# kuldeepbrd1/graspLDM

Hardware: AMD Instinct MI355X
Metric: grasps/sec whole-node (1024-pt cloud, 100 DDIM steps) (higher is better)
Workload: dtype f32 (GEMMs as split-f16 x3 partial products on the f16 matrix pipe, f32 accumulation; GroupNorm / LayerNorm / attention / scheduler in f32); 1 GPU; LDM mode, 256 synthetic 1024-pt clouds per GPU x 20 grasps, 100 DDIM steps: BASELINE.json configs[2] per GPU (configs[3] = this per-GPU workload on 8 GPUs); experiment=fpc, clouds_per_gpu=256, grasps_per_cloud=20, points=1024, ddim_steps=100, encoder=PVCNNEncoder (shipped fpc config), parallelism=cloud-sharded x1, weights=synthetic recipe seed 0, streams=3

## Files before the change

graspldm_amd/csrc/pointwise_mlp.hip:

```cpp
#include "mfma_core.h"

namespace {

struct PwArgs {
  const float *x, *w, *bias, *head_w, *head_b;
  float *y, *z;
  int cin, cout, n, relu, hout, tiles_per_cloud, total_tiles;
  const float *w0, *bias0;
  int cin0;
  int dyn_first;
  int ticket_off;
  int x0_in_planes;
  const float *add;
  long long add_bs, add_rs, add_cs;
  int ranged, rng_off;
  float gain0_r, gain0_b;
  int y_point_major;
  int cin_rows;
};

__global__ __launch_bounds__(512, 2) void pointwise_mlp_kernel(const PwArgs a) {
  constexpr int NC = 32;
  extern __shared__ float lds[];
  const int tid = threadIdx.x, lane = tid & 63;
  const int wave = __builtin_amdgcn_readfirstlane(tid >> 6);
  Ctx c{a.w, lds, tid, wave, lane, 0, 2};
  const int col = lane & 15, kq = lane >> 4;
  const int cblocks = a.cin >> 4, mtiles = a.cout >> 4, mt_per_wave = mtiles >> 3;
  float *zpart = lds + a.cin * NC;
  const WStream hw(a.head_w ? a.head_w : a.w, lane);
  for (int tile = blockIdx.x; tile < a.total_tiles; tile += gridDim.x) {
    const int b = tile / a.tiles_per_cloud, c0 = (tile - b * a.tiles_per_cloud) * NC;
    __syncthreads();
    if (a.w0) {
      float *x0 = zpart + 8 * 16 * NC;
      const float *xb0 = a.x + (size_t)b * a.cin0 * a.n + c0;
      for (int i = tid; i < a.cin0 * 8; i += 512) {
        const int row = i >> 3, q = i & 7;
        *reinterpret_cast<f32x4 *>(x0 + swz<NC>(row, 4 * q)) = *reinterpret_cast<const f32x4 *>(xb0 + (size_t)row * a.n + 4 * q);
      }
      __syncthreads();
      const int cb0 = a.cin0 >> 4, mt_per_wave0 = a.cin >> 7;
      for (int ps = 0; ps < mt_per_wave0; ps += 2) {
        const int mt0 = wave * mt_per_wave0 + ps;
        f32x4 acc[2][2];
#pragma unroll
        for (int mi = 0; mi < 2; ++mi) {
          const f32x4 bv = *reinterpret_cast<const f32x4 *>(a.bias0 + 16 * (mt0 + mi) + 4 * kq);
          acc[mi][0] = bv;
          acc[mi][1] = bv;
        }
        gemm_fast_pf<NC, 4, 1, 2, 2, 2>(c, a.w0, cb0, mt0, 0, x0, acc);
        lds_f *d3 = (lds_f *)lds;
#pragma unroll
        for (int mi = 0; mi < 2; ++mi)
#pragma unroll
          for (int r = 0; r < 4; ++r)
#pragma unroll
            for (int ni = 0; ni < 2; ++ni)
              d3[swz<NC>(16 * (mt0 + mi) + 4 * kq + r, 16 * ni + col)] = fmaxf(acc[mi][ni][r], 0.f);
      }
    } else {
      const float *xb = a.x + (size_t)b * a.cin * a.n + c0;
      for (int i = tid; i < a.cin * 8; i += 512) {
        const int row = i >> 3, q = i & 7;
        const f32x4 v = *reinterpret_cast<const f32x4 *>(xb + (size_t)row * a.n + 4 * q);
        *reinterpret_cast<f32x4 *>(lds + swz<NC>(row, 4 * q)) = v;
      }
    }
    __syncthreads();
    f32x4 zacc[2] = {f32x4{0.f, 0.f, 0.f, 0.f}, f32x4{0.f, 0.f, 0.f, 0.f}};
    for (int ps = 0; ps < mt_per_wave; ps += 2) {
      const int mt0 = wave * mt_per_wave + ps;
      f32x4 acc[2][2];
#pragma unroll
      for (int mi = 0; mi < 2; ++mi) {
        const f32x4 bv = *reinterpret_cast<const f32x4 *>(a.bias + 16 * (mt0 + mi) + 4 * kq);
        acc[mi][0] = bv;
        acc[mi][1] = bv;
      }
      if ((cblocks & 3) == 0) gemm_fast_pf<NC, 4, 1, 2, 2, 4>(c, a.w, cblocks, mt0, 0, lds, acc);
      else gemm_fast_pf<NC, 4, 1, 2, 2, 2>(c, a.w, cblocks, mt0, 0, lds, acc);
#pragma unroll
      for (int mi = 0; mi < 2; ++mi) {
        if (a.relu) {
#pragma unroll
          for (int ni = 0; ni < 2; ++ni)
#pragma unroll
            for (int r = 0; r < 4; ++r) acc[mi][ni][r] = fmaxf(acc[mi][ni][r], 0.f);
        }
        if (a.y) {
          float *yb = a.y + ((size_t)b * a.cout + 16 * (mt0 + mi) + 4 * kq) * a.n + c0 + col;
#pragma unroll
          for (int r = 0; r < 4; ++r)
#pragma unroll
            for (int ni = 0; ni < 2; ++ni) __builtin_nontemporal_store(acc[mi][ni][r], yb + (size_t)r * a.n + 16 * ni);
        }
        if (a.head_w) {
          const f32x4 ah = hw[(size_t)(mt0 + mi) * 64];
#pragma unroll
          for (int r = 0; r < 4; ++r)
#pragma unroll
            for (int ni = 0; ni < 2; ++ni)
              zacc[ni] = __builtin_amdgcn_mfma_f32_16x16x4f32(ah[r], acc[mi][ni][r], zacc[ni], 0, 0, 0);
        }
      }
    }
    if (a.head_w) {
#pragma unroll
      for (int ni = 0; ni < 2; ++ni)
#pragma unroll
        for (int r = 0; r < 4; ++r) zpart[(wave * 16 + 4 * kq + r) * NC + 16 * ni + col] = zacc[ni][r];
      __syncthreads();
      for (int i = tid; i < a.hout * NC; i += 512) {
        const int row = i / NC, cc = i - row * NC;
        float v = a.head_b ? a.head_b[row] : 0.f;
#pragma unroll
        for (int w8 = 0; w8 < 8; ++w8) v += zpart[(w8 * 16 + row) * NC + cc];
        a.z[((size_t)b * a.hout + row) * a.n + c0 + cc] = v;
      }
    }
  }
}

template <int NC>
__device__ __forceinline__ int pw_swz(int row, int col) { return row * NC + (col < 32 ? (col ^ ((row & 1) << 4)) : col); }
template <int NC>
__device__ __forceinline__ void store_planes4_pw(float *planes, int c0, int n, float v0, float v1, float v2, float v3) {
  unsigned h0, h1, l0, l1;
  split_f16x2(v0, v1, h0, l0);
  split_f16x2(v2, v3, h1, l1);
  const int a = ((((c0 >> 5) * kSplit) * 4 + ((c0 >> 3) & 3)) * NC + n) * 4 + ((c0 >> 2) & 1) * 2;
  lds_u2 *d = (lds_u2 *)(planes + a);
  d[0] = u32x2_t{h0, h1};
  d[8 * NC] = u32x2_t{l0, l1};
}

template <int KB0, int NT>
__device__ __forceinline__ void pw_front_split(const WStream &w0s, const float *bias0, const float *x0, float *planes,
                                               int wave, int lane, int mt_per_wave0, bool x0_in_planes, float bsc, float osc) {
  constexpr int NC = 16 * NT;
  const int col = lane & 15, kq = lane >> 4;
  u32x4 bp[KB0][NT][kSplit];
#pragma unroll
  for (int kb = 0; kb < KB0; ++kb)
#pragma unroll
    for (int ni = 0; ni < NT; ++ni) {
      float v[8];
#pragma unroll
      for (int j = 0; j < 8; ++j) v[j] = x0[pw_swz<NC>(32 * kb + 8 * kq + j, 16 * ni + col)] * bsc;
      split_planes8(v, bp[kb][ni]);
    }
  if (x0_in_planes) __syncthreads();
  u32x4 af[2][KB0][kSplit];
  const int mt_first = wave * mt_per_wave0, mt_last = mt_first + mt_per_wave0 - 2;
  auto load_a = [&](int mi, int kb, int mt0) {
#pragma unroll
    for (int pl = 0; pl < kSplit; ++pl) af[mi][kb][pl] = w0s.raw_at(((mt0 + mi) * KB0 + kb) * kFragBytes, pl * 1024);
  };
#pragma unroll
  for (int mi = 0; mi < 2; ++mi)
#pragma unroll
    for (int kb = 0; kb < KB0; ++kb) load_a(mi, kb, mt_first);
  for (int mt0 = mt_first; mt0 <= mt_last; mt0 += 2) {
    const int mtn = mt0 + 2 <= mt_last ? mt0 + 2 : mt_last;
    f32x4 acc[2][NT];
#pragma unroll
    for (int mi = 0; mi < 2; ++mi) {
      const f32x4 bv = *reinterpret_cast<const f32x4 *>(bias0 + 16 * (mt0 + mi) + 4 * kq) * bsc;
#pragma unroll
      for (int ni = 0; ni < NT; ++ni) acc[mi][ni] = bv;
    }
#pragma unroll
    for (int mi = 0; mi < 2; ++mi)
#pragma unroll
      for (int kb = 0; kb < KB0; ++kb) {
#pragma unroll
        for (int ni = 0; ni < NT; ++ni) acc[mi][ni] = mfma_split(af[mi][kb], bp[kb][ni], acc[mi][ni]);
        __builtin_amdgcn_sched_barrier(0);
        load_a(mi, kb, mtn);
        __builtin_amdgcn_sched_barrier(0);
      }
#pragma unroll
    for (int mi = 0; mi < 2; ++mi)
#pragma unroll
      for (int ni = 0; ni < NT; ++ni)
        store_planes4_pw<NC>(planes, 16 * (mt0 + mi) + 4 * kq, 16 * ni + col, fmaxf(acc[mi][ni][0], 0.f) * osc,
                             fmaxf(acc[mi][ni][1], 0.f) * osc, fmaxf(acc[mi][ni][2], 0.f) * osc, fmaxf(acc[mi][ni][3], 0.f) * osc);
  }
}

#ifdef GLDM_DEBUG_KNOBS
__device__ long long g_pw_stamp[64];
#define GLDM_PW_STAMP(i) \
  do { if (blockIdx.x == 5 && tile == 5 + 2 * (int)gridDim.x && (threadIdx.x & 63) == 0 && (wave == 0 || wave == 7)) \
         g_pw_stamp[(wave ? 32 : 0) + (i)] = (long long)__builtin_readcyclecounter(); } while (0)
#else
#define GLDM_PW_STAMP(i) do {} while (0)
#endif
template <bool ADD, int NT, int MU = 2>
__global__ __launch_bounds__(512, 2) void pointwise_mlp_sp_kernel(const PwArgs a) {
  constexpr int NC = 16 * NT;
  extern __shared__ float lds[];
  const int tid = threadIdx.x, lane = tid & 63;
  const int wave = __builtin_amdgcn_readfirstlane(tid >> 6);
  const int col = lane & 15, kq = lane >> 4;
  const int kb32 = a.cin >> 5, mtiles = a.cout >> 4;
  float *planes = lds;
  float *zpart = lds;
  float *zdyn = lds + a.cin * (NC / 2) * kSplit;
  float *x0 = a.x0_in_planes ? lds : zdyn;
  int *ticket = (int *)(lds + a.ticket_off);
  const WStream hw(a.head_w ? a.head_w : a.w, lane);
  const WStream wv(a.w, lane);
  const lds_u4 *pl3 = (const lds_u4 *)planes + kq * NC + col;
  for (int tile = blockIdx.x; tile < a.total_tiles; tile += gridDim.x) {
    const int b = tile / a.tiles_per_cloud, c0 = (tile - b * a.tiles_per_cloud) * NC;
    const int ntv = min(NT, (a.n - c0) >> 4);
    __syncthreads();
    GLDM_PW_STAMP(0);
    if (tid == 0) *ticket = a.dyn_first;
    float s_main = 1.0f;
    float *rng = lds + a.rng_off;
    auto range_publish = [&](float mx) {
      mx = half_max(row_pair_max(row16_max(mx)));
      if (lane == 0) rng[wave] = mx;
    };
    auto range_read = [&]() {
      const f32x4 r0 = *reinterpret_cast<const f32x4 *>(rng), r1 = *reinterpret_cast<const f32x4 *>(rng + 4);
      const float mx = fmaxf(fmaxf(fmaxf(r0[0], r0[1]), fmaxf(r0[2], r0[3])), fmaxf(fmaxf(r1[0], r1[1]), fmaxf(r1[2], r1[3])));
      return __uint_as_float(__builtin_amdgcn_readfirstlane(__float_as_uint(mx)));
    };
    if (a.w0) {
      const float *xb0 = a.x + (size_t)b * a.cin0 * a.n + c0;
      float mx = 0.f;
      for (int i = tid; i < a.cin0 * (NC / 4); i += 512) {
        const int row = i / (NC / 4), q = i - row * (NC / 4);
        f32x4 v = f32x4{0.f, 0.f, 0.f, 0.f};
        if (4 * q < 16 * ntv) v = *reinterpret_cast<const f32x4 *>(xb0 + (size_t)row * a.n + 4 * q);
        *reinterpret_cast<f32x4 *>(x0 + pw_swz<NC>(row, 4 * q)) = v;
        mx = fmaxf(fmaxf(mx, fmaxf(fabsf(v[0]), fabsf(v[1]))), fmaxf(fabsf(v[2]), fabsf(v[3])));
      }
      if (a.ranged) range_publish(mx);
      __syncthreads();
      GLDM_PW_STAMP(1);
      float bsc = 1.0f, osc = 1.0f;
      if (a.ranged) {
        const float m0 = range_read(), s0 = range_pow2(m0);
        s_main = range_pow2(a.gain0_r * m0 + a.gain0_b);
        bsc = pow2_inv(s0);
        osc = s0 * pow2_inv(s_main);
      }
      const int mt_per_wave0 = a.cin >> 7;
      const WStream w0s(a.w0, lane);
      switch (a.cin0 >> 5) {
        case 1: pw_front_split<1, NT>(w0s, a.bias0, x0, planes, wave, lane, mt_per_wave0, a.x0_in_planes != 0, bsc, osc); break;
        case 2: pw_front_split<2, NT>(w0s, a.bias0, x0, planes, wave, lane, mt_per_wave0, a.x0_in_planes != 0, bsc, osc); break;
        default: pw_front_split<3, NT>(w0s, a.bias0, x0, planes, wave, lane, mt_per_wave0, a.x0_in_planes != 0, bsc, osc); break;
      }
    } else {
      const float *xb = a.x + (size_t)b * a.cin_rows * a.n + c0;
      constexpr int kHold = 2;
      const int items = (a.cin >> 3) * NC;
      auto stage_store = [&](int i, float (&v)[8], float inv) {
        const int kg = i / NC, scol = i - kg * NC, row = 8 * kg;
#pragma unroll
        for (int j = 0; j < 8; ++j) v[j] *= inv;
        u32x4 pl[kSplit];
        split_planes8(v, pl);
        lds_u4 *d = (lds_u4 *)planes + (((row >> 5) * kSplit) * 4 + ((row >> 3) & 3)) * NC + scol;
        d[0] = pl[0];
        d[4 * NC] = pl[1];
      };
      auto stage_load = [&](int i, float (&v)[8]) {
        const int kg = i / NC, scol = i - kg * NC, row = 8 * kg;
        const bool in = scol < 16 * ntv && row < a.cin_rows;
#pragma unroll
        for (int j = 0; j < 8; ++j) v[j] = in ? xb[(size_t)(row + j) * a.n + scol] : 0.f;
      };
      if (NT == 2 && a.ranged && items <= kHold * 512) {
        float hv[kHold][8];
        float mx = 0.f;
#pragma unroll
        for (int q = 0; q < kHold; ++q) {
          const int i = tid + 512 * q;
          if (i < items) {
            stage_load(i, hv[q]);
#pragma unroll
            for (int j = 0; j < 8; ++j) mx = fmaxf(mx, fabsf(hv[q][j]));
          }
        }
        range_publish(mx);
        __syncthreads();
        s_main = range_pow2(range_read());
        const float inv = pow2_inv(s_main);
#pragma unroll
        for (int q = 0; q < kHold; ++q) {
          const int i = tid + 512 * q;
          if (i < items) stage_store(i, hv[q], inv);
        }
      } else {
        float inv = 1.0f;
        if (a.ranged) {
          float mx = 0.f;
          for (int i = tid; i < items; i += 512) {
            float v[8];
            stage_load(i, v);
#pragma unroll
            for (int j = 0; j < 8; ++j) mx = fmaxf(mx, fabsf(v[j]));
          }
          range_publish(mx);
          __syncthreads();
          s_main = range_pow2(range_read());
          inv = pow2_inv(s_main);
        }
        for (int i = tid; i < items; i += 512) {
          float v[8];
          stage_load(i, v);
          stage_store(i, v, inv);
        }
      }
    }
    GLDM_PW_STAMP(2);
    __syncthreads();
    GLDM_PW_STAMP(3);
    f32x4 zacc[NT];
#pragma unroll
    for (int ni = 0; ni < NT; ++ni) zacc[ni] = f32x4{0.f, 0.f, 0.f, 0.f};
    const int units = mtiles / MU;
    u32x4 af[4][MU][kSplit];
    auto load_a = [&](int buf, int mt0, int kb) {
#pragma unroll
      for (int mi = 0; mi < MU; ++mi)
#pragma unroll
        for (int pl = 0; pl < kSplit; ++pl) af[buf][mi][pl] = wv.raw_at(((mt0 + mi) * kb32 + kb) * kFragBytes, pl * 1024);
    };
    u32x4 bs[2][NT][kSplit];
    auto load_b = [&](int buf, int kb) {
#pragma unroll
      for (int ni = 0; ni < NT; ++ni)
#pragma unroll
        for (int pl = 0; pl < kSplit; ++pl) bs[buf][ni][pl] = pl3[(kb * kSplit + pl) * 4 * NC + 16 * ni];
    };
    auto draw = [&]() {
      int t = 0;
      if (lane == 0) t = __hip_atomic_fetch_add(ticket, 1, __ATOMIC_RELAXED, __HIP_MEMORY_SCOPE_WORKGROUP);
      return __builtin_amdgcn_readfirstlane(t);
    };
    const int dyn_first = a.dyn_first;
    int unit = wave;
#pragma unroll
    for (int u = 0; u < 4; ++u) load_a(u, MU * (unit < units ? unit : 0), u);
    load_b(0, 0);
    while (unit < units) {
      const int mt0 = MU * unit;
      const int nxt = unit + 8 < dyn_first ? unit + 8 : draw();
      const int mtn = MU * (nxt < units ? nxt : unit);
      f32x4 acc[MU][NT], bv[MU], ah[MU];
#pragma unroll
      for (int mi = 0; mi < MU; ++mi) {
        bv[mi] = *reinterpret_cast<const f32x4 *>(a.bias + 16 * (mt0 + mi) + 4 * kq);
        ah[mi] = hw[(size_t)(a.head_w ? mt0 + mi : 0) * 64];
#pragma unroll
        for (int ni = 0; ni < NT; ++ni) acc[mi][ni] = f32x4{0.f, 0.f, 0.f, 0.f};
      }
      for (int kb0 = 0; kb0 < kb32; kb0 += 4) {
        const bool tail = kb0 + 4 >= kb32;
#pragma unroll
        for (int u = 0; u < 4; ++u) {
          const int kb = kb0 + u;
          load_b((u + 1) & 1, kb + 1 < kb32 ? kb + 1 : 0);
          __builtin_amdgcn_sched_barrier(0);
#pragma unroll
          for (int mi = 0; mi < MU; ++mi)
#pragma unroll
            for (int ni = 0; ni < NT; ++ni) acc[mi][ni] = mfma_split(af[u][mi], bs[u & 1][ni], acc[mi][ni]);
          __builtin_amdgcn_sched_barrier(0);
          load_a(u, tail ? mtn : mt0, tail ? u : kb + 4);
        }
      }
#pragma unroll
      for (int mi = 0; mi < MU; ++mi) {
#pragma unroll
        for (int ni = 0; ni < NT; ++ni)
#pragma unroll
          for (int r = 0; r < 4; ++r) {
            float v = __builtin_fmaf(acc[mi][ni][r], s_main, bv[mi][r]);
            if constexpr (ADD)
              v += a.add[(long long)b * a.add_bs + (long long)(16 * (mt0 + mi) + 4 * kq + r) * a.add_rs +
                         (long long)(c0 + (ni < ntv ? 16 * ni + col : col)) * a.add_cs];
            acc[mi][ni][r] = a.relu ? fmaxf(v, 0.f) : v;
          }
        if (a.y && a.y_point_major) {
          float *yb = a.y + ((size_t)b * a.n + c0 + col) * a.cout + 16 * (mt0 + mi) + 4 * kq;
#pragma unroll
          for (int ni = 0; ni < NT; ++ni)
            if (ni < ntv) *reinterpret_cast<f32x4 *>(yb + (size_t)16 * ni * a.cout) = acc[mi][ni];
        } else if (a.y) {
          float *yb = a.y + ((size_t)b * a.cout + 16 * (mt0 + mi) + 4 * kq) * a.n + c0 + col;
#pragma unroll
          for (int r = 0; r < 4; ++r)
#pragma unroll
            for (int ni = 0; ni < NT; ++ni)
              if (ni < ntv) __builtin_nontemporal_store(acc[mi][ni][r], yb + (size_t)r * a.n + 16 * ni);
        }
      }
      if (a.head_w) {
        const bool drawn = unit >= dyn_first;
        f32x4 zu[NT];
#pragma unroll
        for (int ni = 0; ni < NT; ++ni) zu[ni] = drawn ? f32x4{0.f, 0.f, 0.f, 0.f} : zacc[ni];
#pragma unroll
        for (int mi = 0; mi < MU; ++mi) {
#pragma unroll
          for (int r = 0; r < 4; ++r)
#pragma unroll
            for (int ni = 0; ni < NT; ++ni)
              zu[ni] = __builtin_amdgcn_mfma_f32_16x16x4f32(ah[mi][r], acc[mi][ni][r], zu[ni], 0, 0, 0);
        }
        if (drawn) {
          float *slot = zdyn + (unit - dyn_first) * a.hout * NC;
#pragma unroll
          for (int r = 0; r < 4; ++r)
            if (4 * kq + r < a.hout) {
#pragma unroll
              for (int ni = 0; ni < NT; ++ni) slot[(4 * kq + r) * NC + 16 * ni + col] = zu[ni][r];
            }
        } else {
#pragma unroll
          for (int ni = 0; ni < NT; ++ni) zacc[ni] = zu[ni];
        }
      }
      unit = nxt;
    }
    GLDM_PW_STAMP(16);
    if (a.head_w) {
      __syncthreads();
      GLDM_PW_STAMP(17);
#pragma unroll
      for (int ni = 0; ni < NT; ++ni)
#pragma unroll
        for (int r = 0; r < 4; ++r) zpart[(wave * 16 + 4 * kq + r) * NC + 16 * ni + col] = zacc[ni][r];
      __syncthreads();
      const int nd = units - dyn_first;
      for (int i0 = 0; i0 < a.hout * NC * 4; i0 += 512) {
        const int i = i0 + tid, o = i >> 2, p = i & 3;
        const bool live = o < a.hout * NC;
        const int row = live ? o / NC : 0, cc = live ? o - row * NC : 0;
        float v = zpart[((2 * p) * 16 + row) * NC + cc] + zpart[((2 * p + 1) * 16 + row) * NC + cc];
        for (int d = p; d < nd; d += 4) v += zdyn[(d * a.hout + row) * NC + cc];
        v += dpp_mov<0xB1>(v);
        v += dpp_mov<0x4E>(v);
        if (live && p == 0 && cc < 16 * ntv) a.z[((size_t)b * a.hout + row) * a.n + c0 + cc] = v + (a.head_b ? a.head_b[row] : 0.f);
      }
    }
    GLDM_PW_STAMP(18);
  }
}

using gldm_dev::cu_count;

struct PwPlan {
  int cin;
  int mu, nt;
  int dyn_first, ticket_off, x0_in_planes;
  size_t lds_bytes;
};

int plan_pointwise(bool split_f16, int cin0, int cin_arg, int cout, int n, int hout, bool add, bool y_point_major, PwPlan &p) {
  if (cin0 < 0 || cin_arg <= 0 || cout <= 0 || n <= 0 || hout < 0 || hout > 16) return GLDM_ERR_UNSUPPORTED;
  if ((y_point_major || add) && !split_f16) return GLDM_ERR_UNSUPPORTED;
  const bool front = cin0 > 0, head = hout > 0;
  const int cin = (split_f16 && !front && (cin_arg & 7) == 0) ? (cin_arg + 127) & ~127 : cin_arg;
  const int mu = (split_f16 && !front && !head && cout < 256 && ((size_t)cin * 32 * 2 * kSplit + 64) * 2 <= (size_t)160 * 1024) ? 1 : 2;
  if ((cin & 31) || (split_f16 ? (n & 15) : (n & 31)) || (split_f16 ? (cout & (16 * mu - 1)) : (cout & 255))) return GLDM_ERR_UNSUPPORTED;
  if ((front || head) && (cout & 255)) return GLDM_ERR_UNSUPPORTED;
  if (front && ((cin0 & 31) || (cin & 255))) return GLDM_ERR_UNSUPPORTED;
  size_t lds_bytes = ((size_t)cin * 32 + 8 * 16 * 32 + (size_t)cin0 * 32) * sizeof(float);
  if (split_f16) {
    if (cin & 127) return GLDM_ERR_UNSUPPORTED;
    if (cin0 > 96) return GLDM_ERR_UNSUPPORTED;
  }
  int dyn_first = 0, ticket_off = 0, nt = 2, x0_in_planes = 0;
  if (split_f16) {
    const size_t cap = (size_t)160 * 1024 - 64;
    const int units = cout / (16 * mu);
    auto plan = [&](int ncol, bool x0_under, size_t &planes, size_t &region, int &first) {
      planes = (size_t)cin * ncol * 2 * kSplit;
      region = (front && !x0_under) ? (size_t)cin0 * ncol * sizeof(float) : 0;
      if (planes + region > cap) return false;
      if (x0_under && (size_t)cin0 * ncol * sizeof(float) > planes) return false;
      int drawn = units > 8 ? units - 8 : 0;
      if (head) {
        const size_t slot = (size_t)hout * ncol * sizeof(float);
        const int room = (int)((cap - planes) / slot);
        if (drawn > room) drawn = room;
        if (planes < (size_t)8 * 16 * ncol * sizeof(float)) drawn = 0;
      }
      first = (units - drawn + 7) & ~7;
      if (head && (size_t)(units - first) * hout * ncol * sizeof(float) > region)
        region = (size_t)(units - first) * hout * ncol * sizeof(float);
      return planes + region <= cap;
    };
    size_t planes = 0, region = 0;
    if (!plan(32, false, planes, region, dyn_first)) return GLDM_ERR_UNSUPPORTED;
    if ((planes + region + 64) * 2 > (size_t)160 * 1024 && n >= 48) {
      size_t p3 = 0, r3 = 0;
      int f3 = 0;
      if (plan(48, front, p3, r3, f3)) {
        nt = 3; planes = p3; region = r3; dyn_first = f3; x0_in_planes = front ? 1 : 0;
      }
    }
    ticket_off = (int)((planes + region) / sizeof(float));
    lds_bytes = planes + region + 64;
  }
  if (lds_bytes > 160 * 1024) return GLDM_ERR_UNSUPPORTED;
  p = PwPlan{cin, mu, nt, dyn_first, ticket_off, x0_in_planes, lds_bytes};
  return GLDM_OK;
}

int launch_pointwise(const float *x, const float *w0, const float *b0, int cin0, const float *w, const float *bias, int b,
                     int cin_arg, int cout, int n, int relu, const float *head_w, const float *head_b, int hout, float *y,
                     float *z, hipStream_t stream, bool split_f16 = false, const float *add = nullptr, long long add_bs = 0,
                     long long add_rs = 0, long long add_cs = 0, const float *front_gain = nullptr, bool y_point_major = false) {
  if (y_point_major && !y) return GLDM_ERR_UNSUPPORTED;
  if (!x || !w || !bias || b <= 0 || cin_arg <= 0 || cout <= 0 || n <= 0) return GLDM_ERR_INVALID_ARG;
  if (!y && !head_w) return GLDM_ERR_INVALID_ARG;
  if (head_w && (!z || hout <= 0 || hout > 16)) return GLDM_ERR_INVALID_ARG;
  if (w0 && (!b0 || cin0 <= 0)) return GLDM_ERR_UNSUPPORTED;
  PwPlan p{};
  const int rc = plan_pointwise(split_f16, w0 ? cin0 : 0, cin_arg, cout, n, head_w ? hout : 0, add != nullptr, y_point_major, p);
  if (rc != GLDM_OK) return rc;
  const int cin_rows = cin_arg, cin = p.cin, mu = p.mu, nt = p.nt;
  const size_t lds_bytes = p.lds_bytes;
  PwArgs a{};
  a.x = x; a.w = w; a.bias = bias; a.head_w = head_w; a.head_b = head_b; a.y = y; a.z = z;
  a.cin = cin; a.cout = cout; a.n = n; a.relu = relu; a.hout = hout;
  a.w0 = w0; a.bias0 = b0; a.cin0 = cin0;
  a.dyn_first = p.dyn_first; a.ticket_off = p.ticket_off; a.x0_in_planes = p.x0_in_planes;
  a.add = add; a.add_bs = add_bs; a.add_rs = add_rs; a.add_cs = add_cs;
  a.y_point_major = y_point_major ? 1 : 0;
  a.cin_rows = cin_rows;
  a.rng_off = p.ticket_off + 4;
  a.ranged = split_f16 && (!w0 || front_gain);
  if (w0 && front_gain) {
    a.gain0_r = front_gain[0]; a.gain0_b = front_gain[1];
    if (!(a.gain0_r >= 0.f) || !(a.gain0_b >= 0.f)) return GLDM_ERR_INVALID_ARG;
  }
  a.tiles_per_cloud = (n + 16 * nt - 1) / (16 * nt);
  a.total_tiles = b * a.tiles_per_cloud;
  const int per_cu = lds_bytes * 2 <= 160 * 1024 ? 2 : 1;
  int grid = cu_count() * per_cu;
  if (grid > a.total_tiles) grid = a.total_tiles;
  const dim3 g(grid), t(512);
  constexpr int kLim = 160 * 1024;
  using gldm_dev::launch_dynamic_lds;
  if (split_f16 && mu == 1 && nt == 2) {
    if (add) launch_dynamic_lds<pointwise_mlp_sp_kernel<true, 2, 1>>(g, t, kLim, lds_bytes, stream, a);
    else launch_dynamic_lds<pointwise_mlp_sp_kernel<false, 2, 1>>(g, t, kLim, lds_bytes, stream, a);
  } else if (split_f16 && add && nt == 3) launch_dynamic_lds<pointwise_mlp_sp_kernel<true, 3>>(g, t, kLim, lds_bytes, stream, a);
  else if (split_f16 && nt == 3) launch_dynamic_lds<pointwise_mlp_sp_kernel<false, 3>>(g, t, kLim, lds_bytes, stream, a);
  else if (split_f16 && add) launch_dynamic_lds<pointwise_mlp_sp_kernel<true, 2>>(g, t, kLim, lds_bytes, stream, a);
  else if (split_f16) launch_dynamic_lds<pointwise_mlp_sp_kernel<false, 2>>(g, t, kLim, lds_bytes, stream, a);
  else launch_dynamic_lds<pointwise_mlp_kernel>(g, t, kLim, lds_bytes, stream, a);
#ifdef GLDM_DEBUG_KNOBS
  if (split_f16 && getenv("GLDM_PW_STAMP")) {
    long long h[64];
    (void)hipStreamSynchronize(stream);
    (void)hipMemcpyFromSymbol(h, HIP_SYMBOL(g_pw_stamp), sizeof(h));
    for (int w = 0; w < 2; ++w) {
      const long long *q = h + 32 * w;
      printf("pointwise split %d(%d)->%d b=%d wave %d: stage %lld front %lld barrier %lld |", cin, cin0, cout, b, w ? 7 : 0,
             q[1] - q[0], q[2] - q[1], q[3] - q[2]);
      printf(" main %lld wait %lld head %lld total %lld\n", q[16] - q[3], q[17] - q[16], q[18] - q[17], q[18] - q[0]);
    }
  }
#endif
  return hipGetLastError() == hipSuccess ? GLDM_OK : GLDM_ERR_LAUNCH;
}
}

GLDM_API int gldm_pointwise_mlp_supported(int split_f16, int cin0, int cin, int cout, int n, int hout, int with_addend,
                                          int point_major) {
  PwPlan p{};
  return plan_pointwise(split_f16 != 0, cin0, cin, cout, n, hout, with_addend != 0, point_major != 0, p);
}

GLDM_API int gldm_pointwise_mlp(const float *x, const float *w_packed, const float *bias, int b, int cin, int cout,
                                int n, int relu, const float *head_w_packed, const float *head_bias, int hout,
                                float *y, float *z, gldm_stream_t stream) {
  return launch_pointwise(x, nullptr, nullptr, 0, w_packed, bias, b, cin, cout, n, relu, head_w_packed, head_bias, hout,
                          y, z, reinterpret_cast<hipStream_t>(stream));
}

GLDM_API int gldm_pointwise_mlp2(const float *x, const float *w0_packed, const float *bias0, int cin0,
                                 const float *w_packed, const float *bias, int b, int cin, int cout, int n,
                                 const float *head_w_packed, const float *head_bias, int hout, float *y, float *z,
                                 gldm_stream_t stream) {
  if (!w0_packed) return GLDM_ERR_INVALID_ARG;
  return launch_pointwise(x, w0_packed, bias0, cin0, w_packed, bias, b, cin, cout, n, 1, head_w_packed, head_bias,
                          hout, y, z, reinterpret_cast<hipStream_t>(stream));
}

GLDM_API int gldm_pointwise_mlp_f16x2(const float *x, const float *w_split, const float *bias, int b, int cin, int cout,
                                       int n, int relu, const float *head_w_packed, const float *head_bias, int hout,
                                       float *y, float *z, gldm_stream_t stream) {
  return launch_pointwise(x, nullptr, nullptr, 0, w_split, bias, b, cin, cout, n, relu, head_w_packed, head_bias, hout,
                          y, z, reinterpret_cast<hipStream_t>(stream), true);
}

GLDM_API int gldm_pointwise_mlp_f16x2_pm(const float *x, const float *w_split, const float *bias, int b, int cin, int cout,
                                          int n, int relu, float *y_point_major, gldm_stream_t stream) {
  return launch_pointwise(x, nullptr, nullptr, 0, w_split, bias, b, cin, cout, n, relu, nullptr, nullptr, 0, y_point_major,
                          nullptr, reinterpret_cast<hipStream_t>(stream), true, nullptr, 0, 0, 0, nullptr, true);
}

GLDM_API int gldm_pointwise_mlp_f16x2_add(const float *x, const float *w_split, const float *bias, const float *add,
                                           long long add_cloud_stride, long long add_row_stride, long long add_col_stride, int b,
                                           int cin, int cout, int n, int relu, float *y, gldm_stream_t stream) {
  if (!add) return GLDM_ERR_INVALID_ARG;
  return launch_pointwise(x, nullptr, nullptr, 0, w_split, bias, b, cin, cout, n, relu, nullptr, nullptr, 0, y, nullptr,
                          reinterpret_cast<hipStream_t>(stream), true, add, add_cloud_stride, add_row_stride, add_col_stride);
}

GLDM_API int gldm_pointwise_mlp2_f16x2(const float *x, const float *w0_packed, const float *bias0, int cin0,
                                        const float *w_split, const float *bias, int b, int cin, int cout, int n,
                                        const float *head_w_packed, const float *head_bias, int hout,
                                        const float *front_gain, float *y, float *z, gldm_stream_t stream) {
  if (!w0_packed) return GLDM_ERR_INVALID_ARG;
  return launch_pointwise(x, w0_packed, bias0, cin0, w_split, bias, b, cin, cout, n, 1, head_w_packed, head_bias,
                          hout, y, z, reinterpret_cast<hipStream_t>(stream), true, nullptr, 0, 0, 0, front_gain);
}
```

Baseline: 306,700 grasps/s.

## Prefetch next tile's front-layer input into registers and pre-split planes

The first-layer input for the next tile is now loaded from global memory into registers at the end of the current tile, so the load latency overlaps with the head reduction. The input is split into f16 hi/lo planes once when written to LDS, instead of each wave re-splitting swizzled f32 values in the front GEMM. Barriers are reordered so the first weight-fragment loads are issued before the synchronisation. This costs extra registers (16 floats per thread) in a kernel already bounded at 512 threads x 2 blocks, which may cause spills. The non-ranged path drops a barrier, which is only safe if the planes write is ordered by the later sync.

```diff
diff --git a/graspldm_amd/csrc/pointwise_mlp.hip b/graspldm_amd/csrc/pointwise_mlp.hip
--- a/graspldm_amd/csrc/pointwise_mlp.hip
+++ b/graspldm_amd/csrc/pointwise_mlp.hip
@@ -124,8 +124,6 @@
 }
 
 template <int NC>
-__device__ __forceinline__ int pw_swz(int row, int col) { return row * NC + (col < 32 ? (col ^ ((row & 1) << 4)) : col); }
-template <int NC>
 __device__ __forceinline__ void store_planes4_pw(float *planes, int c0, int n, float v0, float v1, float v2, float v3) {
   unsigned h0, h1, l0, l1;
   split_f16x2(v0, v1, h0, l0);
@@ -141,17 +139,6 @@
                                                int wave, int lane, int mt_per_wave0, bool x0_in_planes, float bsc, float osc) {
   constexpr int NC = 16 * NT;
   const int col = lane & 15, kq = lane >> 4;
-  u32x4 bp[KB0][NT][kSplit];
-#pragma unroll
-  for (int kb = 0; kb < KB0; ++kb)
-#pragma unroll
-    for (int ni = 0; ni < NT; ++ni) {
-      float v[8];
-#pragma unroll
-      for (int j = 0; j < 8; ++j) v[j] = x0[pw_swz<NC>(32 * kb + 8 * kq + j, 16 * ni + col)] * bsc;
-      split_planes8(v, bp[kb][ni]);
-    }
-  if (x0_in_planes) __syncthreads();
   u32x4 af[2][KB0][kSplit];
   const int mt_first = wave * mt_per_wave0, mt_last = mt_first + mt_per_wave0 - 2;
   auto load_a = [&](int mi, int kb, int mt0) {
@@ -162,6 +149,16 @@
   for (int mi = 0; mi < 2; ++mi)
 #pragma unroll
     for (int kb = 0; kb < KB0; ++kb) load_a(mi, kb, mt_first);
+  __syncthreads();
+  u32x4 bp[KB0][NT][kSplit];
+  const lds_u4 *xp = (const lds_u4 *)x0 + kq * NC + col;
+#pragma unroll
+  for (int kb = 0; kb < KB0; ++kb)
+#pragma unroll
+    for (int ni = 0; ni < NT; ++ni)
+#pragma unroll
+      for (int pl = 0; pl < kSplit; ++pl) bp[kb][ni][pl] = xp[(kb * kSplit + pl) * 4 * NC + 16 * ni];
+  if (x0_in_planes) __syncthreads();
   for (int mt0 = mt_first; mt0 <= mt_last; mt0 += 2) {
     const int mtn = mt0 + 2 <= mt_last ? mt0 + 2 : mt_last;
     f32x4 acc[2][NT];
@@ -214,6 +211,23 @@
   const WStream hw(a.head_w ? a.head_w : a.w, lane);
   const WStream wv(a.w, lane);
   const lds_u4 *pl3 = (const lds_u4 *)planes + kq * NC + col;
+  constexpr int kFrontHold = 2;
+  const int front_items = a.w0 ? (a.cin0 >> 3) * NC : 0;
+  float fx[kFrontHold][8];
+  auto front_load = [&](int t, bool go) {
+    const int tb = t / a.tiles_per_cloud, tc0 = (t - tb * a.tiles_per_cloud) * NC;
+    const int tntv = min(NT, (a.n - tc0) >> 4);
+    const float *xb0 = a.x + (size_t)tb * a.cin0 * a.n + tc0;
+#pragma unroll
+    for (int q = 0; q < kFrontHold; ++q) {
+      const int i = tid + 512 * q;
+      const int kg = i / NC, scol = i - kg * NC;
+      const bool in = go && i < front_items && scol < 16 * tntv;
+#pragma unroll
+      for (int j = 0; j < 8; ++j) fx[q][j] = in ? xb0[(size_t)(8 * kg + j) * a.n + scol] : 0.f;
+    }
+  };
+  front_load(blockIdx.x, a.w0 && (int)blockIdx.x < a.total_tiles);
   for (int tile = blockIdx.x; tile < a.total_tiles; tile += gridDim.x) {
     const int b = tile / a.tiles_per_cloud, c0 = (tile - b * a.tiles_per_cloud) * NC;
     const int ntv = min(NT, (a.n - c0) >> 4);
@@ -232,25 +246,35 @@
       return __uint_as_float(__builtin_amdgcn_readfirstlane(__float_as_uint(mx)));
     };
     if (a.w0) {
-      const float *xb0 = a.x + (size_t)b * a.cin0 * a.n + c0;
       float mx = 0.f;
-      for (int i = tid; i < a.cin0 * (NC / 4); i += 512) {
-        const int row = i / (NC / 4), q = i - row * (NC / 4);
-        f32x4 v = f32x4{0.f, 0.f, 0.f, 0.f};
-        if (4 * q < 16 * ntv) v = *reinterpret_cast<const f32x4 *>(xb0 + (size_t)row * a.n + 4 * q);
-        *reinterpret_cast<f32x4 *>(x0 + pw_swz<NC>(row, 4 * q)) = v;
-        mx = fmaxf(fmaxf(mx, fmaxf(fabsf(v[0]), fabsf(v[1]))), fmaxf(fabsf(v[2]), fabsf(v[3])));
-      }
-      if (a.ranged) range_publish(mx);
-      __syncthreads();
-      GLDM_PW_STAMP(1);
+#pragma unroll
+      for (int q = 0; q < kFrontHold; ++q)
+#pragma unroll
+        for (int j = 0; j < 8; ++j) mx = fmaxf(mx, fabsf(fx[q][j]));
       float bsc = 1.0f, osc = 1.0f;
       if (a.ranged) {
+        range_publish(mx);
+        __syncthreads();
         const float m0 = range_read(), s0 = range_pow2(m0);
         s_main = range_pow2(a.gain0_r * m0 + a.gain0_b);
         bsc = pow2_inv(s0);
         osc = s0 * pow2_inv(s_main);
       }
+#pragma unroll
+      for (int q = 0; q < kFrontHold; ++q) {
+        const int i = tid + 512 * q;
+        if (i < front_items) {
+          const int kg = i / NC, scol = i - kg * NC;
+#pragma unroll
+          for (int j = 0; j < 8; ++j) fx[q][j] *= bsc;
+          u32x4 pl[kSplit];
+          split_planes8(fx[q], pl);
+          lds_u4 *d = (lds_u4 *)x0 + (((kg >> 2) * kSplit) * 4 + (kg & 3)) * NC + scol;
+          d[0] = pl[0];
+          d[4 * NC] = pl[1];
+        }
+      }
+      GLDM_PW_STAMP(1);
       const int mt_per_wave0 = a.cin >> 7;
       const WStream w0s(a.w0, lane);
       switch (a.cin0 >> 5) {
@@ -321,9 +345,6 @@
         }
       }
     }
-    GLDM_PW_STAMP(2);
-    __syncthreads();
-    GLDM_PW_STAMP(3);
     f32x4 zacc[NT];
 #pragma unroll
     for (int ni = 0; ni < NT; ++ni) zacc[ni] = f32x4{0.f, 0.f, 0.f, 0.f};
@@ -351,6 +372,9 @@
     int unit = wave;
 #pragma unroll
     for (int u = 0; u < 4; ++u) load_a(u, MU * (unit < units ? unit : 0), u);
+    GLDM_PW_STAMP(2);
+    __syncthreads();
+    GLDM_PW_STAMP(3);
     load_b(0, 0);
     while (unit < units) {
       const int mt0 = MU * unit;
@@ -434,6 +458,7 @@
       unit = nxt;
     }
     GLDM_PW_STAMP(16);
+    front_load(tile + gridDim.x, a.w0 && tile + (int)gridDim.x < a.total_tiles);
     if (a.head_w) {
       __syncthreads();
       GLDM_PW_STAMP(17);
```

Result: no change. 307,700 grasps/s, median of 4 (+0.3%).
